# invictus717/MetaTransformer

Measured on AMD Instinct MI355X. Metric: encoder samples/sec at B=256,N=197,C=768 (Base), higher is better.
Workload: dtype bf16; 1 GPU; BASELINE config 2: Meta-Transformer-Base forward+backward+AdamW, tokens [256,197,768] bf16 per GPU, 12L/768d/12h, fp32 master weights, random init N(0,0.02); mode=train, per_gpu_batch=256, global_batch=256, parallelism=single

## Files before the change

### metatransformer_amd/csrc/common.h

```cpp
#pragma once
constexpr int ME_POL_LN_ST = 0;
constexpr int ME_POL_LN_LD = 0;
constexpr int ME_POL_ATTN_ST = 0;
constexpr int ME_POL_SLAB = 0;
#define ME_NT_LOAD(POL, ptr) ((POL) ? __builtin_nontemporal_load(ptr) : *(ptr))
#define ME_NT_STORE(POL, val, ptr) do { if (POL) __builtin_nontemporal_store((val), (ptr)); else *(ptr) = (val); } while (0)
#include <hip/hip_runtime.h>
#include <stdint.h>
#include <stdio.h>
#include "../../include/metaenc.h"

typedef __bf16 bf16_t;
typedef __attribute__((ext_vector_type(8))) __bf16 bf16x8;
typedef __attribute__((ext_vector_type(4))) __bf16 bf16x4;
typedef __attribute__((ext_vector_type(2))) __bf16 bf16x2;
typedef __attribute__((ext_vector_type(16))) float f32x16;
typedef __attribute__((ext_vector_type(4))) float f32x4;
typedef __attribute__((ext_vector_type(2))) float f32x2;
typedef __attribute__((ext_vector_type(4))) uint32_t u32x4;
constexpr float ME_GG8_LO = -0.13f, ME_GG8_STEP = 1.26f / 255.0f;
constexpr int ME_STATS_GROUP = 256;
typedef __attribute__((ext_vector_type(2))) uint32_t u32x2;

#define ME_WAVE 64

void me_set_error(const char* fmt, ...);
#define ME_CHECK_ARG(cond, ...)                 \
    do {                                        \
        if (!(cond)) {                          \
            me_set_error(__VA_ARGS__);          \
            return ME_ERR_ARG;                  \
        }                                       \
    } while (0)
#define ME_CHECK_LAUNCH(name)                                                        \
    do {                                                                             \
        hipError_t e__ = hipGetLastError();                                          \
        if (e__ != hipSuccess) {                                                     \
            me_set_error("%s: launch failed: %s", name, hipGetErrorString(e__));     \
            return ME_ERR_HIP;                                                       \
        }                                                                            \
    } while (0)

struct OncePerDevice {
    bool done[64] = {};
    bool need() {
        int d = 0;
        if (hipGetDevice(&d) != hipSuccess || d < 0 || d >= 64) return true;
        if (done[d]) return false;
        done[d] = true;
        return true;
    }
};

static inline int device_cus() {
    static int n = 0;
// ... 208 lines not shown
```

### metatransformer_amd/csrc/elementwise.hip

```cpp
#include "common.h"

namespace {

constexpr int EW_THREADS = 256;
inline unsigned ew_blocks(int64_t work_items) {
    int64_t b = (work_items + EW_THREADS - 1) / EW_THREADS;
    const int64_t cap = 256 * 8;
    return (unsigned)(b < 1 ? 1 : (b > cap ? cap : b));
}

__device__ __forceinline__ float ld1_any(const void* base, int dt, int64_t i) {
    if (dt == ME_F16) return (float)reinterpret_cast<const _Float16*>(base)[i];
    return load1_as_f32(base, dt, i);
}
__device__ __forceinline__ void st1_any(void* base, int dt, int64_t i, float v) {
    if (dt == ME_F16) reinterpret_cast<_Float16*>(base)[i] = (_Float16)v;
    else store1_from_f32(base, dt, i, v);
}
__global__ __launch_bounds__(EW_THREADS) void cast_any_kernel(const void* __restrict__ src, int sdt, void* __restrict__ dst,
                                                              int ddt, int64_t n) {
    for (int64_t i = (int64_t)blockIdx.x * EW_THREADS + threadIdx.x; i < n; i += (int64_t)gridDim.x * EW_THREADS)
        st1_any(dst, ddt, i, ld1_any(src, sdt, i));
}

// ... 42 lines not shown
        tx_tiles = (b.item[k].cols + 63) / 64;
        const int64_t nt = tx_tiles * ((b.item[k].rows + 63) / 64);
        if (t < nt) break;
        t -= nt;
    }
    if (k >= b.n) return;
    const float* src = reinterpret_cast<const float*>(b.item[k].src);
    uint16_t* dst = reinterpret_cast<uint16_t*>(b.item[k].dst);
    const int64_t rows = b.item[k].rows, cols = b.item[k].cols;
    const int64_t r0 = (t / tx_tiles) * 64, c0 = (t % tx_tiles) * 64;
    const int q = threadIdx.x & 15, p = threadIdx.x >> 4;
#pragma unroll
    for (int pass = 0; pass < 4; ++pass) {
        const int i = p + 16 * pass;
        const int64_t r = r0 + i, c = c0 + 4 * q;
        if (r < rows && c < cols) {
            const f32x4 v = *reinterpret_cast<const f32x4*>(src + r * cols + c);
            if (!transposed) {
                store4_split3(dst + r * 3 * cols, cols, c, v, right_operand != 0);
            } else {
#pragma unroll
                for (int e = 0; e < 4; ++e) tile[i][4 * q + e] = v[e];
            }
        }
    }
    if (!transposed) return;
    __syncthreads();
#pragma unroll
    for (int pass = 0; pass < 4; ++pass) {
        const int i = p + 16 * pass;
        const int64_t c = c0 + i, r = r0 + 4 * q;
        if (c < cols && r < rows)
            store4_split3(dst + c * 3 * rows, rows, r, f32x4{tile[4 * q][i], tile[4 * q + 1][i], tile[4 * q + 2][i], tile[4 * q + 3][i]}, right_operand != 0);
    }
}

__global__ __launch_bounds__(256) void transpose_cast_batched_kernel(const me_tc_batch b) {
    __shared__ float tile[64][65];
    int64_t t = blockIdx.x;
    int k = 0;
    int64_t tx_tiles = 0;
    for (; k < b.n; ++k) {
        tx_tiles = (b.item[k].cols + 63) / 64;
        const int64_t nt = tx_tiles * ((b.item[k].rows + 63) / 64);
        if (t < nt) break;
        t -= nt;
    }
    if (k >= b.n) return;
    const void* src = b.item[k].src;
    void* dst = b.item[k].dst;
    const int64_t rows = b.item[k].rows, cols = b.item[k].cols;
    const int64_t r0 = (t / tx_tiles) * 64, c0 = (t % tx_tiles) * 64;
    const int ssz = b.src_dtype == ME_F32 ? 4 : 2, dsz = b.dst_dtype == ME_F32 ? 4 : 2;
    if (b.src_dtype != ME_F16 && b.dst_dtype != ME_F16 && rows % 4 == 0 && cols % 4 == 0 && (uintptr_t)src % (4 * ssz) == 0 && (uintptr_t)dst % (4 * dsz) == 0) {
        const int q = threadIdx.x & 15, p = threadIdx.x >> 4;
#pragma unroll
        for (int pass = 0; pass < 4; ++pass) {
            const int i = p + 16 * pass;
            const int64_t r = r0 + i, c = c0 + 4 * q;
            const f32x4 v = (r < rows && c < cols) ? load4_as_f32(src, b.src_dtype, r * cols + c) : f32x4{0.f, 0.f, 0.f, 0.f};
#pragma unroll
            for (int e = 0; e < 4; ++e) tile[i][4 * q + e] = v[e];
        }
        __syncthreads();
#pragma unroll
        for (int pass = 0; pass < 4; ++pass) {
            const int i = p + 16 * pass;
            const int64_t c = c0 + i, r = r0 + 4 * q;
            if (c < cols && r < rows) store4_from_f32(dst, b.dst_dtype, c * rows + r, f32x4{tile[4 * q][i], tile[4 * q + 1][i], tile[4 * q + 2][i], tile[4 * q + 3][i]});
        }
        return;
    }
    const int tx = threadIdx.x & 63, ty = threadIdx.x >> 6;
    for (int i = ty; i < 64; i += 4) {
        const int64_t r = r0 + i, c = c0 + tx;
        tile[i][tx] = (r < rows && c < cols) ? ld1_any(src, b.src_dtype, r * cols + c) : 0.f;
    }
    __syncthreads();
    for (int i = ty; i < 64; i += 4) {
        const int64_t c = c0 + i, r = r0 + tx;
        if (c < cols && r < rows) st1_any(dst, b.dst_dtype, c * rows + r, tile[tx][i]);
    }
}

__global__ __launch_bounds__(EW_THREADS) void add_rows_kernel(const void* __restrict__ x, int xdt,
                                                              const void* __restrict__ pos, int pdt, void* __restrict__ y,
                                                              int ydt, int64_t rows, int64_t pos_rows, int cols) {
    const int c4 = cols / 4;
    const int64_t total = rows * c4;
    for (int64_t i = (int64_t)blockIdx.x * EW_THREADS + threadIdx.x; i < total; i += (int64_t)gridDim.x * EW_THREADS) {
        const int64_t r = i / c4;
        const int c = (int)(i % c4) * 4;
        f32x4 v = load4_as_f32(x, xdt, r * cols + c);
        v += load4_as_f32(pos, pdt, (r % pos_rows) * cols + c);
        store4_from_f32(y, ydt, r * cols + c, v);
    }
}

constexpr int CS_SPLITS = 128;
template <typename T> __device__ __forceinline__ f32x4 cs_ld4(const void* base, int64_t idx);
template <> __device__ __forceinline__ f32x4 cs_ld4<float>(const void* base, int64_t idx) {
    return *reinterpret_cast<const f32x4*>(reinterpret_cast<const float*>(base) + idx);
}
template <> __device__ __forceinline__ f32x4 cs_ld4<bf16_t>(const void* base, int64_t idx) {
    const u32x2 raw = *reinterpret_cast<const u32x2*>(reinterpret_cast<const uint16_t*>(base) + idx);
    return f32x4{__uint_as_float(raw[0] << 16), __uint_as_float(raw[0] & 0xffff0000u), __uint_as_float(raw[1] << 16),
// ... 215 lines not shown
        if (pe) v += pe[(int64_t)l * C + c];
        store1_from_f32(out, odt, tok * C + c, v);
    }
}


__global__ __launch_bounds__(EW_THREADS) void dropout_add_kernel(const void* __restrict__ v, int vdt,
                                                                 const void* __restrict__ res, int rdt,
                                                                 void* __restrict__ out, int odt, int64_t rows, int cols,
                                                                 int64_t rows_per_sample, float p_drop, float p_path,
                                                                 uint64_t seed, const float* __restrict__ colscale) {
    const int c4 = cols / 4;
    const int64_t total = rows * c4;
    const float inv_keep = p_drop > 0.f ? 1.0f / (1.0f - p_drop) : 1.0f;
    const float inv_path = p_path > 0.f ? 1.0f / (1.0f - p_path) : 1.0f;
    for (int64_t i = (int64_t)blockIdx.x * EW_THREADS + threadIdx.x; i < total; i += (int64_t)gridDim.x * EW_THREADS) {
        const int64_t r = i / c4;
        const int c = (int)(i % c4) * 4;
        float rowscale = 1.0f;
        if (p_path > 0.f) {
            const uint64_t sample = (uint64_t)(r / rows_per_sample);
            rowscale = u01_hash(seed ^ 0xD1B54A32D192ED03ull, sample) >= p_path ? inv_path : 0.0f;
        }
        f32x4 x = load4_as_f32(v, vdt, r * cols + c);
#pragma unroll
        for (int e = 0; e < 4; ++e) {
            float k = rowscale;
            if (p_drop > 0.f) k = u01_hash(seed, (uint64_t)(r * cols + c + e)) >= p_drop ? k * inv_keep : 0.0f;
            x[e] *= k;
        }
        if (colscale) x *= *reinterpret_cast<const f32x4*>(colscale + c);
        if (res) x += load4_as_f32(res, rdt, r * cols + c);
        store4_from_f32(out, odt, r * cols + c, x);
    }
}

__device__ __forceinline__ float adamw_update(float& pi, float gi, float& mi, float& vi, float lr, float b1, float b2, float eps, float wd,
                                              float bc1, float bc2_sqrt) {
    pi *= (1.0f - lr * wd);
    mi = b1 * mi + (1.0f - b1) * gi;
    vi = b2 * vi + (1.0f - b2) * gi * gi;
    const float denom = sqrtf(vi) / bc2_sqrt + eps;
    pi -= (lr / bc1) * (mi / denom);
    return pi;
}
template <bool VEC>
__global__ __launch_bounds__(EW_THREADS) void adamw_kernel(float* __restrict__ p, const float* __restrict__ g,
                                                           float* __restrict__ m, float* __restrict__ v, int64_t n, float lr,
                                                           float b1, float b2, float eps, float wd, float bc1, float bc2_sqrt,
                                                           float gscale, bf16_t* __restrict__ mirror) {
    if (VEC) {
        const int64_t n4 = n / 4;
        for (int64_t i = (int64_t)blockIdx.x * EW_THREADS + threadIdx.x; i < n4; i += (int64_t)gridDim.x * EW_THREADS) {
            f32x4 pv = *reinterpret_cast<const f32x4*>(p + i * 4), mv = *reinterpret_cast<const f32x4*>(m + i * 4),
                  vv = *reinterpret_cast<const f32x4*>(v + i * 4);
            const f32x4 gv = *reinterpret_cast<const f32x4*>(g + i * 4);
#pragma unroll
            for (int e = 0; e < 4; ++e) {
                float pi = pv[e], mi = mv[e], vi = vv[e];
                adamw_update(pi, gv[e] * gscale, mi, vi, lr, b1, b2, eps, wd, bc1, bc2_sqrt);
                pv[e] = pi; mv[e] = mi; vv[e] = vi;
            }
            *reinterpret_cast<f32x4*>(m + i * 4) = mv;
            *reinterpret_cast<f32x4*>(v + i * 4) = vv;
            *reinterpret_cast<f32x4*>(p + i * 4) = pv;
            if (mirror) {
                bf16x4 o;
#pragma unroll
                for (int e = 0; e < 4; ++e) o[e] = (bf16_t)pv[e];
                *reinterpret_cast<bf16x4*>(mirror + i * 4) = o;
            }
        }
        if (blockIdx.x != 0 || (int64_t)threadIdx.x >= n - n4 * 4) return;
        const int64_t i = n4 * 4 + threadIdx.x;
        float pi = p[i], mi = m[i], vi = v[i];
        adamw_update(pi, g[i] * gscale, mi, vi, lr, b1, b2, eps, wd, bc1, bc2_sqrt);
        m[i] = mi; v[i] = vi; p[i] = pi;
        if (mirror) mirror[i] = (bf16_t)pi;
        return;
    }
    for (int64_t i = (int64_t)blockIdx.x * EW_THREADS + threadIdx.x; i < n; i += (int64_t)gridDim.x * EW_THREADS) {
        float pi = p[i], mi = m[i], vi = v[i];
        adamw_update(pi, g[i] * gscale, mi, vi, lr, b1, b2, eps, wd, bc1, bc2_sqrt);
        m[i] = mi;
        v[i] = vi;
        p[i] = pi;
        if (mirror) mirror[i] = (bf16_t)pi;
    }
}

constexpr int GS_BLOCKS = 1024;
__global__ __launch_bounds__(EW_THREADS) void grad_stats_kernel(const float* __restrict__ g, int64_t n, double* __restrict__ part) {
    double ss = 0.0;
    float bad = 0.f;
    const int64_t n4 = n / 4;
    for (int64_t i = (int64_t)blockIdx.x * EW_THREADS + threadIdx.x; i < n4; i += (int64_t)gridDim.x * EW_THREADS) {
        const f32x4 v = *reinterpret_cast<const f32x4*>(g + i * 4);
#pragma unroll
        for (int e = 0; e < 4; ++e) {
            const bool nf = (__float_as_uint(v[e]) & 0x7f800000u) == 0x7f800000u;
            const double d = nf ? 0.0 : (double)v[e];
            ss = __builtin_fma(d, d, ss);
            bad += nf ? 1.f : 0.f;
        }
    }
    if (blockIdx.x == 0 && threadIdx.x < (int)(n - n4 * 4)) {
        const float v = g[n4 * 4 + threadIdx.x];
        const bool nf = (__float_as_uint(v) & 0x7f800000u) == 0x7f800000u;
        const double d = nf ? 0.0 : (double)v;
        ss = __builtin_fma(d, d, ss);
        bad += nf ? 1.f : 0.f;
    }
    __shared__ double sh[2][EW_THREADS / 64];
    double dss = ss, dbad = bad;
#pragma unroll
    for (int o = 32; o > 0; o >>= 1) { dss += __shfl_xor(dss, o, 64); dbad += __shfl_xor(dbad, o, 64); }
    if ((threadIdx.x & 63) == 0) { sh[0][threadIdx.x >> 6] = dss; sh[1][threadIdx.x >> 6] = dbad; }
// ... 723 lines not shown
```

### metatransformer_amd/csrc/layernorm.hip

```cpp
#include "common.h"
#include <atomic>
#include <type_traits>

namespace {

constexpr int LN_THREADS = 256;
constexpr int LN_MAX_VEC = 16;

template <typename T> __device__ __forceinline__ f32x4 ld4(const void* base, int64_t idx);
template <> __device__ __forceinline__ f32x4 ld4<float>(const void* base, int64_t idx) {
    return ME_NT_LOAD(ME_POL_LN_LD, reinterpret_cast<const f32x4*>(reinterpret_cast<const float*>(base) + idx));
}
template <> __device__ __forceinline__ f32x4 ld4<bf16_t>(const void* base, int64_t idx) {
    const u32x2 raw = ME_NT_LOAD(ME_POL_LN_LD, reinterpret_cast<const u32x2*>(reinterpret_cast<const uint16_t*>(base) + idx));
    return f32x4{__uint_as_float(raw[0] << 16), __uint_as_float(raw[0] & 0xffff0000u), __uint_as_float(raw[1] << 16),
                 __uint_as_float(raw[1] & 0xffff0000u)};
}
template <typename T> __device__ __forceinline__ void st4(void* base, int64_t idx, f32x4 v);
template <> __device__ __forceinline__ void st4<float>(void* base, int64_t idx, f32x4 v) {
    ME_NT_STORE(ME_POL_LN_ST, v, reinterpret_cast<f32x4*>(reinterpret_cast<float*>(base) + idx));
}
template <> __device__ __forceinline__ void st4<bf16_t>(void* base, int64_t idx, f32x4 v) {
    bf16x4 o;
    o[0] = (bf16_t)v[0]; o[1] = (bf16_t)v[1]; o[2] = (bf16_t)v[2]; o[3] = (bf16_t)v[3];
    ME_NT_STORE(ME_POL_LN_ST, __builtin_bit_cast(u32x2, o), reinterpret_cast<u32x2*>(reinterpret_cast<uint16_t*>(base) + idx));
}

struct me_split3_tag {};

constexpr int ln_rows_per_wave(int vpl) { return vpl <= 4 ? 2 : 1; }
template <int VPL, typename TX, typename TY>
__global__ __launch_bounds__(LN_THREADS) void ln_fwd_kernel(const void* __restrict__ x, const float* __restrict__ gamma,
                                                            const float* __restrict__ beta, void* __restrict__ y,
                                                            float* __restrict__ mean_out, float* __restrict__ rstd_out,
                                                            int64_t rows, int C, float eps) {
    constexpr int LN_R = ln_rows_per_wave(VPL);
    const int lane = threadIdx.x & 63;
    const int64_t row0 = ((int64_t)blockIdx.x * (LN_THREADS / 64) + (threadIdx.x >> 6)) * LN_R;
    if (row0 >= rows) return;
    f32x4 v[LN_R][VPL], g[VPL], b[VPL];
#pragma unroll
    for (int r = 0; r < LN_R; ++r) {
        const int64_t row = row0 + r < rows ? row0 + r : rows - 1;
#pragma unroll
        for (int i = 0; i < VPL; ++i) v[r][i] = ld4<TX>(x, row * C + (int64_t)(lane + 64 * i) * 4);
    }
#pragma unroll
    for (int i = 0; i < VPL; ++i) {
        g[i] = *reinterpret_cast<const f32x4*>(gamma + (lane + 64 * i) * 4);
        b[i] = *reinterpret_cast<const f32x4*>(beta + (lane + 64 * i) * 4);
    }
    float mean[LN_R], rstd[LN_R];
#pragma unroll
    for (int r = 0; r < LN_R; ++r) {
        float s = 0.f;
#pragma unroll
        for (int i = 0; i < VPL; ++i) s += (v[r][i][0] + v[r][i][1]) + (v[r][i][2] + v[r][i][3]);
        mean[r] = wave_sum(s) / (float)C;
    }
#pragma unroll
    for (int r = 0; r < LN_R; ++r) {
        float q = 0.f;
#pragma unroll
        for (int i = 0; i < VPL; ++i) {
#pragma unroll
            for (int e = 0; e < 4; ++e) {
                const float d = v[r][i][e] - mean[r];
                q += d * d;
            }
        }
        rstd[r] = rsqrtf(wave_sum(q) / (float)C + eps);
    }
#pragma unroll
    for (int r = 0; r < LN_R; ++r) {
        const int64_t row = row0 + r;
        if (row >= rows) break;
        if (lane == 0) {
            if (mean_out) mean_out[row] = mean[r];
// ... 94 lines not shown
    const int lane = threadIdx.x & 63;
    const int64_t row = (int64_t)blockIdx.x * (LN_THREADS / 64) + (threadIdx.x >> 6);
    if (row >= rows) return;
    float s = 0.f;
    for (int c = lane; c < C; c += 64) s += load1_as_f32(x, x_dt, row * C + c);
    const float mean = wave_sum(s) / (float)C;
    float q = 0.f;
    for (int c = lane; c < C; c += 64) {
        const float d = load1_as_f32(x, x_dt, row * C + c) - mean;
        q += d * d;
    }
    const float rstd = rsqrtf(wave_sum(q) / (float)C + eps);
    if (lane == 0) {
        if (mean_out) mean_out[row] = mean;
        if (rstd_out) rstd_out[row] = rstd;
    }
    for (int c = lane; c < C; c += 64)
        store1_from_f32(y, y_dt, row * C + c, (load1_as_f32(x, x_dt, row * C + c) - mean) * rstd * gamma[c] + beta[c]);
}


constexpr int LNB_BLOCKS = 1024;

template <int VPL, typename TX, typename TDY, bool RES>
__global__ __launch_bounds__(LN_THREADS) void ln_bwd_kernel(const void* __restrict__ dy, int dy_dt,
                                                            const void* __restrict__ x, int x_dt,
                                                            const float* __restrict__ mean,
                                                            const float* __restrict__ rstd,
                                                            const float* __restrict__ gamma,
                                                            const void* __restrict__ dres, int dres_dt,
                                                            void* __restrict__ dx, int dx_dt,
                                                            float* __restrict__ partial, int want_affine,
                                                            int64_t rows, int C) {
    extern __shared__ __attribute__((aligned(16))) float lds_red[];
    const int lane = threadIdx.x & 63, w = threadIdx.x >> 6;
    const int gw = blockIdx.x * (LN_THREADS / 64) + w;
    f32x4 g[VPL], dg[VPL], db[VPL];
#pragma unroll
    for (int i = 0; i < VPL; ++i) {
        g[i] = *reinterpret_cast<const f32x4*>(gamma + (lane + 64 * i) * 4);
        dg[i] = f32x4{0.f, 0.f, 0.f, 0.f};
        db[i] = f32x4{0.f, 0.f, 0.f, 0.f};
    }
    const int64_t nwaves = (int64_t)gridDim.x * (LN_THREADS / 64);
    for (int64_t row0 = gw; row0 < rows; row0 += 2 * nwaves) {
        const int64_t row1 = row0 + nwaves;
        const bool has1 = row1 < rows;
        const int64_t r1 = has1 ? row1 : row0;
        const float mu0 = mean[row0], rs0 = rstd[row0], mu1 = mean[r1], rs1 = rstd[r1];
        f32x4 xh0[VPL], d0[VPL], xh1[VPL], d1[VPL], q0[VPL], q1[VPL];
#pragma unroll
        for (int i = 0; i < VPL; ++i) {
            const int64_t c = (int64_t)(lane + 64 * i) * 4;
            xh0[i] = ld4<TX>(x, row0 * C + c);
            d0[i] = ld4<TDY>(dy, row0 * C + c);
            xh1[i] = ld4<TX>(x, r1 * C + c);
            d1[i] = ld4<TDY>(dy, r1 * C + c);
            if (RES) {
                q0[i] = ld4<TX>(dres, row0 * C + c);
                q1[i] = ld4<TX>(dres, r1 * C + c);
            } else {
                q0[i] = f32x4{0.f, 0.f, 0.f, 0.f};
                q1[i] = q0[i];
            }
        }
        float a0 = 0.f, b0 = 0.f, a1 = 0.f, b1 = 0.f;
        const float w1 = has1 ? 1.0f : 0.0f;
#pragma unroll
        for (int i = 0; i < VPL; ++i) {
#pragma unroll
            for (int e = 0; e < 4; ++e) {
                xh0[i][e] = (xh0[i][e] - mu0) * rs0;
                xh1[i][e] = (xh1[i][e] - mu1) * rs1;
                const float ge0 = d0[i][e] * g[i][e], ge1 = d1[i][e] * g[i][e];
                a0 += ge0; b0 += ge0 * xh0[i][e];
                a1 += ge1; b1 += ge1 * xh1[i][e];
                dg[i][e] += d0[i][e] * xh0[i][e] + w1 * d1[i][e] * xh1[i][e];
                db[i][e] += d0[i][e] + w1 * d1[i][e];
            }
        }
#pragma unroll
        for (int o = 32; o > 0; o >>= 1) {
            a0 += __shfl_xor(a0, o, 64); b0 += __shfl_xor(b0, o, 64);
            a1 += __shfl_xor(a1, o, 64); b1 += __shfl_xor(b1, o, 64);
        }
        const float inv = 1.0f / (float)C;
        a0 *= inv; b0 *= inv; a1 *= inv; b1 *= inv;
#pragma unroll
        for (int i = 0; i < VPL; ++i) {
            const int64_t c = (int64_t)(lane + 64 * i) * 4;
            f32x4 o0, o1;
#pragma unroll
            for (int e = 0; e < 4; ++e) {
                o0[e] = rs0 * (d0[i][e] * g[i][e] - a0 - xh0[i][e] * b0) + q0[i][e];
                o1[e] = rs1 * (d1[i][e] * g[i][e] - a1 - xh1[i][e] * b1) + q1[i][e];
            }
            st4<TX>(dx, row0 * C + c, o0);
            if (has1) st4<TX>(dx, row1 * C + c, o1);
        }
    }
    if (want_affine) {
#pragma unroll
        for (int i = 0; i < VPL; ++i) {
            const int c = (lane + 64 * i) * 4;
            *reinterpret_cast<f32x4*>(lds_red + (w * 2 + 0) * C + c) = dg[i];
            *reinterpret_cast<f32x4*>(lds_red + (w * 2 + 1) * C + c) = db[i];
        }
        __syncthreads();
        for (int c = threadIdx.x; c < 2 * C; c += LN_THREADS) {
            const int which = c / C, col = c % C;
            const float v = (lds_red[(0 * 2 + which) * C + col] + lds_red[(1 * 2 + which) * C + col]) +
                            (lds_red[(2 * 2 + which) * C + col] + lds_red[(3 * 2 + which) * C + col]);
            partial[((int64_t)blockIdx.x * 2 + which) * C + col] = v;
        }
    }
}

__global__ __launch_bounds__(1024) void ln_bwd_fold_sets_kernel(const me_ln_fold_batch fb) {
    __shared__ float sh[2][64][65];
    const me_ln_fold_set st = fb.set[blockIdx.y];
    const int C = fb.cols;
    const int cq = threadIdx.x & 15, rs = threadIdx.x >> 4;
    const int c = blockIdx.x * 64 + 4 * cq;
    f32x4 a = {0.f, 0.f, 0.f, 0.f}, b = {0.f, 0.f, 0.f, 0.f};
    if (c < C) {
        for (int r = rs; r < st.nrows; r += 64) {
            a += *reinterpret_cast<const f32x4*>(st.partial + ((int64_t)r * 2 + 0) * C + c);
            b += *reinterpret_cast<const f32x4*>(st.partial + ((int64_t)r * 2 + 1) * C + c);
        }
    }
#pragma unroll
    for (int e = 0; e < 4; ++e) { sh[0][rs][4 * cq + e] = a[e]; sh[1][rs][4 * cq + e] = b[e]; }
    __syncthreads();
    if (threadIdx.x < 128) {
        const int w = threadIdx.x >> 6, col = threadIdx.x & 63, cc = blockIdx.x * 64 + col;
        float t[4] = {0.f, 0.f, 0.f, 0.f};
#pragma unroll
        for (int i = 0; i < 64; i += 4)
#pragma unroll
            for (int e = 0; e < 4; ++e) t[e] += sh[w][i + e][col];
        const float tot = (t[0] + t[1]) + (t[2] + t[3]);
        if (cc < C) {
            float* out = w ? st.dbeta : st.dgamma;
            out[cc] = st.accumulate ? out[cc] + tot : tot;
        }
    }
}

__global__ __launch_bounds__(LN_THREADS) void ln_bwd_generic_dx_kernel(const void* __restrict__ dy, int dy_dt,
                                                                       const void* __restrict__ x, int x_dt,
                                                                       const float* __restrict__ mean,
                                                                       const float* __restrict__ rstd,
                                                                       const float* __restrict__ gamma,
                                                                       const void* __restrict__ dres, int dres_dt,
                                                                       void* __restrict__ dx, int dx_dt,
                                                                       int64_t rows, int C) {
    const int lane = threadIdx.x & 63;
    const int64_t row = (int64_t)blockIdx.x * (LN_THREADS / 64) + (threadIdx.x >> 6);
    if (row >= rows) return;
    const float mu = mean[row], rs = rstd[row];
    float s1 = 0.f, s2 = 0.f;
    for (int c = lane; c < C; c += 64) {
        const float xh = (load1_as_f32(x, x_dt, row * C + c) - mu) * rs;
        const float ge = load1_as_f32(dy, dy_dt, row * C + c) * gamma[c];
        s1 += ge;
        s2 += ge * xh;
    }
    const float m1 = wave_sum(s1) / (float)C, m2 = wave_sum(s2) / (float)C;
    for (int c = lane; c < C; c += 64) {
        const float xh = (load1_as_f32(x, x_dt, row * C + c) - mu) * rs;
        const float ge = load1_as_f32(dy, dy_dt, row * C + c) * gamma[c];
        float o = rs * (ge - m1 - xh * m2);
        if (dres) o += load1_as_f32(dres, dres_dt, row * C + c);
        store1_from_f32(dx, dx_dt, row * C + c, o);
    }
}

__global__ __launch_bounds__(256) void ln_bwd_generic_affine_kernel(const void* __restrict__ dy, int dy_dt,
                                                                    const void* __restrict__ x, int x_dt,
                                                                    const float* __restrict__ mean,
                                                                    const float* __restrict__ rstd,
                                                                    float* __restrict__ dgamma,
                                                                    float* __restrict__ dbeta, int64_t rows, int C,
                                                                    int accumulate) {
    __shared__ float sh[2][4][64];
    const int lane = threadIdx.x & 63, w = threadIdx.x >> 6;
    const int c = blockIdx.x * 64 + lane;
    float a = 0.f, b = 0.f;
    if (c < C) {
        for (int64_t r = w; r < rows; r += 4) {
            const float d = load1_as_f32(dy, dy_dt, r * C + c);
            a += d * (load1_as_f32(x, x_dt, r * C + c) - mean[r]) * rstd[r];
            b += d;
        }
    }
    sh[0][w][lane] = a;
// ... 73 lines not shown
    }
#undef LN_ST_CASE
    ME_CHECK_LAUNCH("me_row_stats");
    return ME_OK;
}

extern "C" size_t me_row_stats_partial_bytes(int64_t rows, int cols) {
    return rows > 0 && cols > 0 ? (size_t)(cols / ME_STATS_GROUP) * (size_t)rows * 2 * sizeof(float) : 0;
}

extern "C" int me_row_stats_combine(const float* partials, int64_t rows, int cols, float eps, float* out, void* stream_) {
    hipStream_t stream = reinterpret_cast<hipStream_t>(stream_);
    ME_CHECK_ARG(partials && out, "me_row_stats_combine: null pointer");
    ME_CHECK_ARG(rows >= 0 && cols > 0 && cols % ME_STATS_GROUP == 0, "me_row_stats_combine: cols must be a positive multiple of 256");
    ME_CHECK_ARG((uintptr_t)partials % 8 == 0 && (uintptr_t)out % 8 == 0, "me_row_stats_combine: 8-byte aligned buffers");
    if (rows == 0) return ME_OK;
    ProfScope prof(ME_PROF_ROW_STATS, ME_F32, rows, cols, 1, stream);
    hipLaunchKernelGGL(row_stats_combine_kernel, dim3((unsigned)((rows + 255) / 256)), dim3(256), 0, stream,
                       reinterpret_cast<const float2*>(partials), cols / ME_STATS_GROUP, rows, 1.0f / (float)cols, eps, out);
    ME_CHECK_LAUNCH("me_row_stats_combine");
    return ME_OK;
}

template <auto KERNEL>
static int ln_bwd_resident_blocks(size_t lds_bytes) {
    static std::atomic<int> cached[64][2] = {};
    int dev = 0;
    (void)hipGetDevice(&dev);
    const bool cacheable = dev >= 0 && dev < 64;
    if (cacheable) {
        const int c = cached[dev][lds_bytes ? 1 : 0].load(std::memory_order_acquire);
        if (c) return c;
    }
    int per_cu = 0, cus = 0;
    if (hipOccupancyMaxActiveBlocksPerMultiprocessor(&per_cu, KERNEL, LN_THREADS, lds_bytes) != hipSuccess || per_cu < 1) per_cu = 2;
    if (hipDeviceGetAttribute(&cus, hipDeviceAttributeMultiprocessorCount, dev) != hipSuccess || cus < 1) cus = 256;
    const int c = per_cu * cus < LNB_BLOCKS ? per_cu * cus : LNB_BLOCKS;
    if (cacheable) cached[dev][lds_bytes ? 1 : 0].store(c, std::memory_order_release);
    return c;
}

extern "C" size_t me_layernorm_bwd_workspace(int cols) {
    return (size_t)LNB_BLOCKS * 2 * (size_t)cols * sizeof(float);
}

int me_ln_bwd_fold_sets(const me_ln_fold_set* sets, int n, int cols, void* stream_) {
    hipStream_t stream = reinterpret_cast<hipStream_t>(stream_);
    me_ln_fold_batch fb;
    fb.cols = cols;
    int k = 0;
    for (int i = 0; i < n; ++i)
        if (sets[i].partial) fb.set[k++] = sets[i];
    if (k == 0) return ME_OK;
    hipLaunchKernelGGL(ln_bwd_fold_sets_kernel, dim3((cols + 63) / 64, k), dim3(1024), 0, stream, fb);
    ME_CHECK_LAUNCH("me_layernorm_bwd(fold)");
    return ME_OK;
}

extern "C" int me_layernorm_bwd(const void* dy, int dy_dtype, const void* x, int x_dtype, const float* mean,
                                const float* rstd, const float* gamma, const void* dres, int dres_dtype, void* dx,
                                int dx_dtype, float* dgamma, float* dbeta, int accumulate_affine, int64_t rows,
                                int cols, void* workspace, void* stream_) {
    return me_ln_bwd_deferred(dy, dy_dtype, x, x_dtype, mean, rstd, gamma, dres, dres_dtype, dx, dx_dtype, dgamma, dbeta, accumulate_affine,
                              rows, cols, workspace, stream_, nullptr);
}

int me_ln_bwd_deferred(const void* dy, int dy_dtype, const void* x, int x_dtype, const float* mean, const float* rstd, const float* gamma,
                       const void* dres, int dres_dtype, void* dx, int dx_dtype, float* dgamma, float* dbeta, int accumulate_affine,
                       int64_t rows, int cols, void* workspace, void* stream_, me_ln_fold_set* defer) {
    hipStream_t stream = reinterpret_cast<hipStream_t>(stream_);
    if (defer) defer->partial = nullptr;
    ProfScope prof(ME_PROF_LN_BWD, x_dtype, rows, cols, 0, stream);
    ME_CHECK_ARG(dy && x && mean && rstd && gamma && dx, "me_layernorm_bwd: null pointer");
    ME_CHECK_ARG(me_dtype_ok(dy_dtype) && me_dtype_ok(x_dtype) && me_dtype_ok(dx_dtype), "me_layernorm_bwd: bad dtype");
    ME_CHECK_ARG((dgamma == nullptr) == (dbeta == nullptr), "me_layernorm_bwd: dgamma/dbeta must both be given or both NULL");
    const int want_affine = dgamma != nullptr;
    ME_CHECK_ARG(!want_affine || workspace, "me_layernorm_bwd: workspace required for dgamma/dbeta");
    if (rows == 0) return ME_OK;
    const bool same_stream_dtype = dx_dtype == x_dtype && (dres == nullptr || dres_dtype == x_dtype);
    if (!(cols % 256 == 0 && cols / 256 <= 8) || !same_stream_dtype) {
        hipLaunchKernelGGL(ln_bwd_generic_dx_kernel, dim3((unsigned)((rows + 3) / 4)), dim3(LN_THREADS), 0, stream, dy,
                           dy_dtype, x, x_dtype, mean, rstd, gamma, dres, dres_dtype, dx, dx_dtype, rows, cols);
        ME_CHECK_LAUNCH("me_layernorm_bwd(generic dx)");
        if (want_affine) {
            hipLaunchKernelGGL(ln_bwd_generic_affine_kernel, dim3((cols + 63) / 64), dim3(256), 0, stream, dy, dy_dtype,
                               x, x_dtype, mean, rstd, dgamma, dbeta, rows, cols, accumulate_affine);
            ME_CHECK_LAUNCH("me_layernorm_bwd(generic affine)");
        }
        return ME_OK;
    }
    float* partial = reinterpret_cast<float*>(workspace);
    const size_t lds_bytes = want_affine ? (size_t)4 * 2 * cols * sizeof(float) : 0;
    int nblocks = LNB_BLOCKS;
#define LN_BWD_LAUNCH(V, TX, TDY)                                                                                 \
    do {                                                                                                          \
        if (dres) {                                                                                               \
            nblocks = ln_bwd_resident_blocks<&ln_bwd_kernel<V, TX, TDY, true>>(lds_bytes);                          \
            hipLaunchKernelGGL((ln_bwd_kernel<V, TX, TDY, true>), dim3(nblocks), dim3(LN_THREADS), lds_bytes, stream, dy, dy_dtype, \
                               x, x_dtype, mean, rstd, gamma, dres, dres_dtype, dx, dx_dtype, partial, want_affine, rows, cols);    \
        } else {                                                                                                  \
            nblocks = ln_bwd_resident_blocks<&ln_bwd_kernel<V, TX, TDY, false>>(lds_bytes);                         \
            hipLaunchKernelGGL((ln_bwd_kernel<V, TX, TDY, false>), dim3(nblocks), dim3(LN_THREADS), lds_bytes, stream, dy, dy_dtype, \
                               x, x_dtype, mean, rstd, gamma, dres, dres_dtype, dx, dx_dtype, partial, want_affine, rows, cols);    \
        }                                                                                                         \
    } while (0)
#define LN_BWD_CASE(V)                                                                                            \
    case V:                                                                                                       \
// ... 20 lines not shown
```

### metatransformer_amd/weight_cache.py

```python
from typing import Optional
import weakref

import torch

from . import ops


def _tensor_version(t: torch.Tensor):
    try:
        return t._version
    except RuntimeError:
        return None


class _WeightCache:
    _live = weakref.WeakSet()
    _pending = {}

    def __init__(self):
        self._table = {}
        self._owner = lambda: None
        _WeightCache._live.add(self)

    def __deepcopy__(self, memo):
        return _WeightCache()

    def __getstate__(self):
        return {}

    def __setstate__(self, state):
        self.__init__()

    def bind(self, blk) -> None:
        if self._owner() is not blk:
            self._owner = weakref.ref(blk)

    def has(self, kind: str, name: str, device) -> bool:
        return (kind, name, device) in self._table

    def weights(self):
        blk = self._owner()
        return {} if blk is None else {"qkv": blk.attn.qkv.weight, "proj": blk.attn.proj.weight, "fc1": blk.mlp.fc1.weight, "fc2": blk.mlp.fc2.weight}

    @staticmethod
    def _key(p: torch.Tensor, dtype):
        epoch = ops.WEIGHT_EPOCH if hasattr(p, "_me_flat") else 0
        return (p.data_ptr(), _tensor_version(p), epoch, p.dtype, p.device, dtype)

    @classmethod
    def _scan(cls, kind: str, device, *, missing: bool, dtype=None, src_dtype=None, contiguous: bool = False):
        todo = []
        for c in list(cls._live):
            for n, w in c.weights().items():
                if w.device != device or w.dim() != 2 or src_dtype not in (None, w.dtype) or (contiguous and not w.is_contiguous()):
                    continue
                h = c._table.get((kind, n, w.device))
                if h is not None or missing:
                    k = cls._key(w, h[0][-1] if dtype is None else dtype)
                    if h is None or h[0] != k:
                        todo.append((c, n, k, w))
        return todo

    @staticmethod
    def _refresh(kind: str, todo, mine=None):
        groups = {}
        for e in todo:
            groups.setdefault((e[3].dtype, e[2][-1]), []).append(e)
        own = None
        for (_, dtype), entries in groups.items():
            ws = [w.detach().contiguous() for _, _, _, w in entries]
            outs = ops.transpose_cast_many(ws, dtype) if kind == "t" else ops.split3_many(ws, kind == "x3t")
            for e, t in zip(entries, outs):
                c, n, k, w = e
                c._table[(kind, n, w.device)] = (k, t)
                if e is mine:
                    own = t
        return own

    def fwd(self, name: str, p: torch.Tensor, dtype) -> torch.Tensor:
        if p.dtype == dtype:
            return p.detach()
        if dtype == torch.bfloat16:
            flat = getattr(p, "_me_flat", None)
            if flat is not None:
                v = flat.bf16_view(p)
                if v is not None:
                    return v
        k = self._key(p, dtype)
        slot = ("cast", name, p.device)
        hit = self._table.get(slot)
        if hit is None or hit[0] != k:
            hit = (k, ops.cast(p.detach().contiguous(), dtype))
            self._table[slot] = hit
        return hit[1]

    def transposed(self, name: str, p: torch.Tensor, dtype) -> torch.Tensor:
        k = self._key(p, dtype)
        ev = _WeightCache._pending.pop(p.device, None)
        if ev is not None:
            torch.cuda.current_stream(p.device).wait_event(ev)
        hit = self._table.get(("t", name, p.device))
        if hit is not None and hit[0] == k:
            return hit[1]
        todo = self._scan("t", p.device, missing=True, dtype=dtype, src_dtype=p.dtype)
        mine = next((e for e in todo if e[0] is self and e[1] == name and e[2] == k), None)
        if mine is None:
            mine = (self, name, k, p)
            todo.append(mine)
        return self._refresh("t", todo, mine)

    def split3(self, name: str, p: torch.Tensor, transposed: bool) -> torch.Tensor:
        kind = "x3t" if transposed else "x3"
        k = self._key(p, None)
        slot = (kind, name, p.device)
        hit = self._table.get(slot)
        if hit is not None and hit[0] == k:
            return hit[1]
        if p.dtype != torch.float32 or not p.is_contiguous():
            w32 = ops.cast(p.detach().contiguous(), torch.float32)
            w32 = ops.transpose_cast(w32, torch.float32) if transposed else w32
            out = ops.split3(w32, right_operand=True)
            self._table[slot] = (k, out)
            return out
        mine = (self, name, k, p)
        todo = [mine] + [e for e in self._scan(kind, p.device, missing=False, src_dtype=torch.float32, contiguous=True)
                         if not (e[0] is self and e[1] == name)]
        return self._refresh(kind, todo, mine)

    @classmethod
    def prefetch_transposed(cls, device) -> int:
        todo = cls._scan("t", device, missing=False)
        cls._refresh("t", todo)
        if todo:
            ev = torch.cuda.Event()
            ev.record(torch.cuda.current_stream(device))
            cls._pending[device] = ev
        return len(todo)

    def operands(self, weights, cdt, x3: bool, transposed: bool):
        w, wt = {}, ({} if transposed else None)
# ... 24 lines not shown
```

Measured before the change: 8514 samples/s.

## Add bf16 transpose path, nontemporal AdamW/LN-bwd loads, split LN fold kernel

Adds a bf16-to-bf16 transpose path that moves 8 elements per 16-byte access. The weight cache now transposes from the existing bf16 mirror of the fp32 master weights instead of reading fp32. AdamW moment and gradient traffic and the LayerNorm-backward input loads switch to nontemporal loads and stores to limit cache pollution. The LN backward fold kernel is split into smaller 256-thread blocks, one per gamma/beta output, to raise parallelism.

```diff
diff --git a/metatransformer_amd/csrc/common.h b/metatransformer_amd/csrc/common.h
--- a/metatransformer_amd/csrc/common.h
+++ b/metatransformer_amd/csrc/common.h
@@ -1,6 +1,8 @@
 #pragma once
 constexpr int ME_POL_LN_ST = 0;
 constexpr int ME_POL_LN_LD = 0;
+constexpr int ME_POL_LNB_LD = 1;
+constexpr int ME_POL_ADAMW = 1;
 constexpr int ME_POL_ATTN_ST = 0;
 constexpr int ME_POL_SLAB = 0;
 #define ME_NT_LOAD(POL, ptr) ((POL) ? __builtin_nontemporal_load(ptr) : *(ptr))
diff --git a/metatransformer_amd/csrc/elementwise.hip b/metatransformer_amd/csrc/elementwise.hip
--- a/metatransformer_amd/csrc/elementwise.hip
+++ b/metatransformer_amd/csrc/elementwise.hip
@@ -118,6 +118,37 @@
     const int64_t rows = b.item[k].rows, cols = b.item[k].cols;
     const int64_t r0 = (t / tx_tiles) * 64, c0 = (t % tx_tiles) * 64;
     const int ssz = b.src_dtype == ME_F32 ? 4 : 2, dsz = b.dst_dtype == ME_F32 ? 4 : 2;
+    if (b.src_dtype == ME_BF16 && b.dst_dtype == ME_BF16 && rows % 8 == 0 && cols % 8 == 0 && (uintptr_t)src % 16 == 0 && (uintptr_t)dst % 16 == 0) {
+        const int q = threadIdx.x & 7, p = threadIdx.x >> 3;
+        const uint16_t* s16 = reinterpret_cast<const uint16_t*>(src);
+        uint16_t* d16 = reinterpret_cast<uint16_t*>(dst);
+#pragma unroll
+        for (int pass = 0; pass < 2; ++pass) {
+            const int i = p + 32 * pass;
+            const int64_t r = r0 + i, c = c0 + 8 * q;
+            u32x4 raw = {0u, 0u, 0u, 0u};
+            if (r < rows && c < cols) raw = *reinterpret_cast<const u32x4*>(s16 + r * cols + c);
+#pragma unroll
+            for (int e = 0; e < 4; ++e) {
+                tile[i][8 * q + 2 * e] = __uint_as_float(raw[e] << 16);
+                tile[i][8 * q + 2 * e + 1] = __uint_as_float(raw[e] & 0xffff0000u);
+            }
+        }
+        __syncthreads();
+#pragma unroll
+        for (int pass = 0; pass < 2; ++pass) {
+            const int i = p + 32 * pass;
+            const int64_t c = c0 + i, r = r0 + 8 * q;
+            if (c < cols && r < rows) {
+                u32x4 o;
+#pragma unroll
+                for (int e = 0; e < 4; ++e)
+                    o[e] = (__float_as_uint(tile[8 * q + 2 * e][i]) >> 16) | (__float_as_uint(tile[8 * q + 2 * e + 1][i]) & 0xffff0000u);
+                *reinterpret_cast<u32x4*>(d16 + c * rows + r) = o;
+            }
+        }
+        return;
+    }
     if (b.src_dtype != ME_F16 && b.dst_dtype != ME_F16 && rows % 4 == 0 && cols % 4 == 0 && (uintptr_t)src % (4 * ssz) == 0 && (uintptr_t)dst % (4 * dsz) == 0) {
         const int q = threadIdx.x & 15, p = threadIdx.x >> 4;
 #pragma unroll
@@ -439,17 +470,17 @@
     if (VEC) {
         const int64_t n4 = n / 4;
         for (int64_t i = (int64_t)blockIdx.x * EW_THREADS + threadIdx.x; i < n4; i += (int64_t)gridDim.x * EW_THREADS) {
-            f32x4 pv = *reinterpret_cast<const f32x4*>(p + i * 4), mv = *reinterpret_cast<const f32x4*>(m + i * 4),
-                  vv = *reinterpret_cast<const f32x4*>(v + i * 4);
-            const f32x4 gv = *reinterpret_cast<const f32x4*>(g + i * 4);
+            f32x4 pv = *reinterpret_cast<const f32x4*>(p + i * 4), mv = ME_NT_LOAD(ME_POL_ADAMW, reinterpret_cast<const f32x4*>(m + i * 4)),
+                  vv = ME_NT_LOAD(ME_POL_ADAMW, reinterpret_cast<const f32x4*>(v + i * 4));
+            const f32x4 gv = ME_NT_LOAD(ME_POL_ADAMW, reinterpret_cast<const f32x4*>(g + i * 4));
 #pragma unroll
             for (int e = 0; e < 4; ++e) {
                 float pi = pv[e], mi = mv[e], vi = vv[e];
                 adamw_update(pi, gv[e] * gscale, mi, vi, lr, b1, b2, eps, wd, bc1, bc2_sqrt);
                 pv[e] = pi; mv[e] = mi; vv[e] = vi;
             }
-            *reinterpret_cast<f32x4*>(m + i * 4) = mv;
-            *reinterpret_cast<f32x4*>(v + i * 4) = vv;
+            ME_NT_STORE(ME_POL_ADAMW, mv, reinterpret_cast<f32x4*>(m + i * 4));
+            ME_NT_STORE(ME_POL_ADAMW, vv, reinterpret_cast<f32x4*>(v + i * 4));
             *reinterpret_cast<f32x4*>(p + i * 4) = pv;
             if (mirror) {
                 bf16x4 o;
diff --git a/metatransformer_amd/csrc/layernorm.hip b/metatransformer_amd/csrc/layernorm.hip
--- a/metatransformer_amd/csrc/layernorm.hip
+++ b/metatransformer_amd/csrc/layernorm.hip
@@ -7,23 +7,23 @@
 constexpr int LN_THREADS = 256;
 constexpr int LN_MAX_VEC = 16;
 
-template <typename T> __device__ __forceinline__ f32x4 ld4(const void* base, int64_t idx);
-template <> __device__ __forceinline__ f32x4 ld4<float>(const void* base, int64_t idx) {
-    return ME_NT_LOAD(ME_POL_LN_LD, reinterpret_cast<const f32x4*>(reinterpret_cast<const float*>(base) + idx));
-}
-template <> __device__ __forceinline__ f32x4 ld4<bf16_t>(const void* base, int64_t idx) {
-    const u32x2 raw = ME_NT_LOAD(ME_POL_LN_LD, reinterpret_cast<const u32x2*>(reinterpret_cast<const uint16_t*>(base) + idx));
-    return f32x4{__uint_as_float(raw[0] << 16), __uint_as_float(raw[0] & 0xffff0000u), __uint_as_float(raw[1] << 16),
-                 __uint_as_float(raw[1] & 0xffff0000u)};
-}
-template <typename T> __device__ __forceinline__ void st4(void* base, int64_t idx, f32x4 v);
-template <> __device__ __forceinline__ void st4<float>(void* base, int64_t idx, f32x4 v) {
-    ME_NT_STORE(ME_POL_LN_ST, v, reinterpret_cast<f32x4*>(reinterpret_cast<float*>(base) + idx));
-}
-template <> __device__ __forceinline__ void st4<bf16_t>(void* base, int64_t idx, f32x4 v) {
-    bf16x4 o;
-    o[0] = (bf16_t)v[0]; o[1] = (bf16_t)v[1]; o[2] = (bf16_t)v[2]; o[3] = (bf16_t)v[3];
-    ME_NT_STORE(ME_POL_LN_ST, __builtin_bit_cast(u32x2, o), reinterpret_cast<u32x2*>(reinterpret_cast<uint16_t*>(base) + idx));
+template <typename T, int POL = ME_POL_LN_LD> __device__ __forceinline__ f32x4 ld4(const void* base, int64_t idx) {
+    if constexpr (std::is_same<T, float>::value) {
+        return ME_NT_LOAD(POL, reinterpret_cast<const f32x4*>(reinterpret_cast<const float*>(base) + idx));
+    } else {
+        const u32x2 raw = ME_NT_LOAD(POL, reinterpret_cast<const u32x2*>(reinterpret_cast<const uint16_t*>(base) + idx));
+        return f32x4{__uint_as_float(raw[0] << 16), __uint_as_float(raw[0] & 0xffff0000u), __uint_as_float(raw[1] << 16),
+                     __uint_as_float(raw[1] & 0xffff0000u)};
+    }
+}
+template <typename T, int POL = ME_POL_LN_ST> __device__ __forceinline__ void st4(void* base, int64_t idx, f32x4 v) {
+    if constexpr (std::is_same<T, float>::value) {
+        ME_NT_STORE(POL, v, reinterpret_cast<f32x4*>(reinterpret_cast<float*>(base) + idx));
+    } else {
+        bf16x4 o;
+        o[0] = (bf16_t)v[0]; o[1] = (bf16_t)v[1]; o[2] = (bf16_t)v[2]; o[3] = (bf16_t)v[3];
+        ME_NT_STORE(POL, __builtin_bit_cast(u32x2, o), reinterpret_cast<u32x2*>(reinterpret_cast<uint16_t*>(base) + idx));
+    }
 }
 
 struct me_split3_tag {};
@@ -224,13 +224,13 @@
 #pragma unroll
         for (int i = 0; i < VPL; ++i) {
             const int64_t c = (int64_t)(lane + 64 * i) * 4;
-            xh0[i] = ld4<TX>(x, row0 * C + c);
-            d0[i] = ld4<TDY>(dy, row0 * C + c);
-            xh1[i] = ld4<TX>(x, r1 * C + c);
-            d1[i] = ld4<TDY>(dy, r1 * C + c);
+            xh0[i] = ld4<TX, ME_POL_LNB_LD>(x, row0 * C + c);
+            d0[i] = ld4<TDY, ME_POL_LNB_LD>(dy, row0 * C + c);
+            xh1[i] = ld4<TX, ME_POL_LNB_LD>(x, r1 * C + c);
+            d1[i] = ld4<TDY, ME_POL_LNB_LD>(dy, r1 * C + c);
             if (RES) {
-                q0[i] = ld4<TX>(dres, row0 * C + c);
-                q1[i] = ld4<TX>(dres, r1 * C + c);
+                q0[i] = ld4<TX, ME_POL_LNB_LD>(dres, row0 * C + c);
+                q1[i] = ld4<TX, ME_POL_LNB_LD>(dres, r1 * C + c);
             } else {
                 q0[i] = f32x4{0.f, 0.f, 0.f, 0.f};
                 q1[i] = q0[i];
@@ -288,32 +288,31 @@
     }
 }
 
-__global__ __launch_bounds__(1024) void ln_bwd_fold_sets_kernel(const me_ln_fold_batch fb) {
-    __shared__ float sh[2][64][65];
-    const me_ln_fold_set st = fb.set[blockIdx.y];
+constexpr int LN_FOLD_COLS = 16;
+__global__ __launch_bounds__(256) void ln_bwd_fold_sets_kernel(const me_ln_fold_batch fb) {
+    __shared__ float sh[64][LN_FOLD_COLS + 1];
+    const me_ln_fold_set st = fb.set[blockIdx.y >> 1];
+    const int which = blockIdx.y & 1;
     const int C = fb.cols;
-    const int cq = threadIdx.x & 15, rs = threadIdx.x >> 4;
-    const int c = blockIdx.x * 64 + 4 * cq;
-    f32x4 a = {0.f, 0.f, 0.f, 0.f}, b = {0.f, 0.f, 0.f, 0.f};
+    const int cq = threadIdx.x & 3, rs = threadIdx.x >> 2;
+    const int c = blockIdx.x * LN_FOLD_COLS + 4 * cq;
+    f32x4 a = {0.f, 0.f, 0.f, 0.f};
     if (c < C) {
-        for (int r = rs; r < st.nrows; r += 64) {
-            a += *reinterpret_cast<const f32x4*>(st.partial + ((int64_t)r * 2 + 0) * C + c);
-            b += *reinterpret_cast<const f32x4*>(st.partial + ((int64_t)r * 2 + 1) * C + c);
-        }
-    }
-#pragma unroll
-    for (int e = 0; e < 4; ++e) { sh[0][rs][4 * cq + e] = a[e]; sh[1][rs][4 * cq + e] = b[e]; }
+        for (int r = rs; r < st.nrows; r += 64) a += *reinterpret_cast<const f32x4*>(st.partial + ((int64_t)r * 2 + which) * C + c);
+    }
+#pragma unroll
+    for (int e = 0; e < 4; ++e) sh[rs][4 * cq + e] = a[e];
     __syncthreads();
-    if (threadIdx.x < 128) {
-        const int w = threadIdx.x >> 6, col = threadIdx.x & 63, cc = blockIdx.x * 64 + col;
+    if (threadIdx.x < LN_FOLD_COLS) {
+        const int col = threadIdx.x, cc = blockIdx.x * LN_FOLD_COLS + col;
         float t[4] = {0.f, 0.f, 0.f, 0.f};
 #pragma unroll
         for (int i = 0; i < 64; i += 4)
 #pragma unroll
-            for (int e = 0; e < 4; ++e) t[e] += sh[w][i + e][col];
+            for (int e = 0; e < 4; ++e) t[e] += sh[i + e][col];
         const float tot = (t[0] + t[1]) + (t[2] + t[3]);
         if (cc < C) {
-            float* out = w ? st.dbeta : st.dgamma;
+            float* out = which ? st.dbeta : st.dgamma;
             out[cc] = st.accumulate ? out[cc] + tot : tot;
         }
     }
@@ -493,7 +492,7 @@
     for (int i = 0; i < n; ++i)
         if (sets[i].partial) fb.set[k++] = sets[i];
     if (k == 0) return ME_OK;
-    hipLaunchKernelGGL(ln_bwd_fold_sets_kernel, dim3((cols + 63) / 64, k), dim3(1024), 0, stream, fb);
+    hipLaunchKernelGGL(ln_bwd_fold_sets_kernel, dim3((cols + LN_FOLD_COLS - 1) / LN_FOLD_COLS, 2 * k), dim3(256), 0, stream, fb);
     ME_CHECK_LAUNCH("me_layernorm_bwd(fold)");
     return ME_OK;
 }
diff --git a/metatransformer_amd/weight_cache.py b/metatransformer_amd/weight_cache.py
--- a/metatransformer_amd/weight_cache.py
+++ b/metatransformer_amd/weight_cache.py
@@ -65,10 +65,12 @@
     def _refresh(kind: str, todo, mine=None):
         groups = {}
         for e in todo:
-            groups.setdefault((e[3].dtype, e[2][-1]), []).append(e)
+            src = _WeightCache._mirror(e[3], e[2][-1]) if kind == "t" else None
+            src = e[3].detach().contiguous() if src is None else src
+            groups.setdefault((src.dtype, e[2][-1]), []).append((e, src))
         own = None
-        for (_, dtype), entries in groups.items():
-            ws = [w.detach().contiguous() for _, _, _, w in entries]
+        for (_, dtype), pairs in groups.items():
+            entries, ws = [e for e, _ in pairs], [s for _, s in pairs]
             outs = ops.transpose_cast_many(ws, dtype) if kind == "t" else ops.split3_many(ws, kind == "x3t")
             for e, t in zip(entries, outs):
                 c, n, k, w = e
@@ -77,15 +79,17 @@
                     own = t
         return own
 
+    @staticmethod
+    def _mirror(p: torch.Tensor, dtype) -> Optional[torch.Tensor]:
+        view = getattr(getattr(p, "_me_flat", None), "bf16_view", None) if dtype == torch.bfloat16 and p.dtype != dtype else None
+        return None if view is None else view(p)
+
     def fwd(self, name: str, p: torch.Tensor, dtype) -> torch.Tensor:
         if p.dtype == dtype:
             return p.detach()
-        if dtype == torch.bfloat16:
-            flat = getattr(p, "_me_flat", None)
-            if flat is not None:
-                v = flat.bf16_view(p)
-                if v is not None:
-                    return v
+        v = self._mirror(p, dtype)
+        if v is not None:
+            return v
         k = self._key(p, dtype)
         slot = ("cast", name, p.device)
         hit = self._table.get(slot)
```

Result: no change. 8553 samples/s (median of 6 runs) (+0.5%).
